# kyegomez/Kosmos-X

Measured on AMD Instinct MI355X. Metric: multimodal forward samples/sec (224x224 img + 50 tok) @ 24L/2048d, higher is better.
Workload: dtype mixed fp16/f16c (CLIP tower: fp16 MFMA; Perceiver + decoder: fp16 MFMA + fp8-e4m3 correction MFMAs; fp32 accumulate / residual / statistics)

## Files before the change

### include/kosmosx_hip.h

```cpp
#ifndef KOSMOSX_HIP_H
#define KOSMOSX_HIP_H

#include <stddef.h>
#include <stdint.h>

#ifdef __cplusplus
extern "C" {
#endif

#define KX_ABI_VERSION 7

typedef enum {
  KX_OK = 0,
  KX_ERR_INVALID_ARG = 1,
  KX_ERR_WORKSPACE = 2,
  KX_ERR_LAUNCH = 3,
  KX_ERR_UNSUPPORTED = 4
} kx_status;

typedef enum { KX_PREC_BF16 = 0, KX_PREC_F32 = 1, KX_PREC_BF16X3 = 2, KX_PREC_F16C = 3, KX_PREC_F16 = 4, KX_PREC_F32W24 = 5,
               KX_PREC_F32W16 = 6, KX_PREC_F16CHL = 7  } kx_precision;
typedef enum { KX_CORR_BOTH = 0, KX_CORR_WEIGHT = 1, KX_CORR_ACT = 2, KX_CORR_NONE = 3 } kx_f16c_corr;
typedef enum { KX_F32 = 0, KX_BF16 = 1, KX_BF16X3 = 2, KX_F16C = 3, KX_F16 = 4, KX_F16P = 5, KX_F16HL = 6 } kx_dtype;
typedef enum { KX_ACT_NONE = 0, KX_ACT_GELU = 1, KX_ACT_QUICK_GELU = 2, KX_ACT_RELU = 5, KX_ACT_SWISH = 6 } kx_act;
typedef enum { KX_ATTN_FULL = 0, KX_ATTN_CAUSAL = 1 } kx_attn_mask;

int kx_version(void);
int kx_last_error(char* buf, size_t n);


int kx_layernorm(const float* x, const float* pre_add, const float* gamma, const float* beta,
                 void* y, kx_dtype ydt, int64_t rows, int64_t cols, float eps,
                 int64_t rows_per_group, int64_t out_group_stride, int64_t out_row_offset,
                 void* stream);

typedef struct {
  const void* A; int64_t lda;
  const void* W; int64_t ldw;
  void* C; int64_t ldc; int32_t cdt;
  const float* bias;
  const float* residual; int64_t ldr;
  int64_t M, N, K;
  int32_t act;
  float qscale; int64_t qcols;
  const float* xq_cs; const float* xq_ss;
  const float* xk_cs; const float* xk_ss;
  int64_t xpos_T; int64_t xpos_dim;
  int32_t prec;
  int32_t tile;
  const float* row_stats; const float* colsum;
  float* stats_out;
  void* splitk_ws; size_t splitk_ws_bytes; int32_t splitk;
  const float* ln_gamma; const float* ln_beta; float ln_eps;
  const float* stats_partials; int64_t stats_in_nseg; int64_t stats_in_seg; float stats_eps;
  int32_t stats_out_seg;
  void* ln_out; int32_t ln_out_dt; const float* ln_out_gamma; const float* ln_out_beta; float ln_out_eps;
  const uint8_t* w_scale;
  void* ln_operand_out; int32_t ln_operand_dt; float* ln_operand_stats;
  int32_t w_tiled;
  int32_t ksplit; void* C2; const float* residual2; const float* a_add;
  void* pair_ws; size_t pair_ws_bytes;
  float* row_stats_scratch;
  int32_t f16c_corr;
  uint32_t* splitk_flags;
} kx_gemm_args;
int kx_gemm(const kx_gemm_args* args, void* stream);
int kx_pair_split_errors(unsigned* word_out);

typedef struct {
  const void* q; int64_t q_batch_stride; int64_t q_row_stride;
  const void* k; const void* v; int64_t kv_batch_stride; int64_t kv_row_stride;
  void* out; int64_t out_batch_stride; int64_t out_row_stride; int32_t odt;
  int64_t B, H, Tq, Tk;
  int32_t mask;
  int32_t prec;
  float* stats_out;
  float* lse_out;
  float dropout_p; int32_t dropout_site; uint64_t dropout_seed;
} kx_attn_args;
int kx_attention(const kx_attn_args* args, void* stream);

int kx_row_stats_finalize(const float* partials, int64_t rows, int64_t nseg, int64_t seg_size, float eps,
                          float* out, void* stream);

int kx_embed_splice(const int64_t* tokens, const float* embed, const float* pos, const float* img,
                    float* out, int64_t B, int64_t Tt, int64_t n_img, int64_t d, int64_t vocab,
                    int64_t max_pos, int64_t splice_at, int32_t u1_alias, int64_t pos_offset, void* stream);

int kx_token_range(const int64_t* tokens, int64_t n, int64_t* out2, void* stream);


typedef struct {
  uint32_t struct_bytes;
  int32_t do_sample;
  const float* logits; int64_t ld; int64_t B; int64_t V;
  float temperature; int32_t top_k; float top_p; float repetition_penalty;
  uint64_t seed; int64_t position;
  const int64_t* sequence_ids;
  int64_t* history; int64_t hist_ld; int64_t hist_len;
  uint8_t* finished;
  int64_t eos_id; int64_t pad_id;
  int64_t* next_token;
  int64_t* out_tokens; int64_t out_ld; int64_t out_col;
  int32_t* kept_count; uint8_t* keep_mask;
} kx_sample_args;
int kx_sample_logits(const kx_sample_args* args, void* stream);

int kx_embed_step(const int64_t* tokens, const float* embed, const float* pos, float* out, int64_t B, int64_t d,
                  int64_t vocab, int64_t max_pos, int64_t pos_a, int64_t pos_b, void* stream);

typedef enum {
  KX_STRUCT_GEMM_ARGS = 0, KX_STRUCT_ATTN_ARGS = 1, KX_STRUCT_VIT_LAYER = 2, KX_STRUCT_VIT_WEIGHTS = 3,
  KX_STRUCT_PERCEIVER_LAYER = 4, KX_STRUCT_PERCEIVER_WEIGHTS = 5, KX_STRUCT_DECODER_LAYER = 6,
  KX_STRUCT_DECODER_WEIGHTS = 7, KX_STRUCT_RESAMPLE_PLAN = 8, KX_STRUCT_PROF_RECORD = 9, KX_STRUCT_SAMPLE_ARGS = 10,
  KX_STRUCT_COUNT = 11
} kx_struct_id;
size_t kx_struct_bytes(int32_t id);
typedef struct {
  const float *ln1_g, *ln1_b;
  const void* wqkv; const float* bqkv;
  const void* wo;   const float* bo;
  const float *ln2_g, *ln2_b;
  const void* w1;   const float* b1;
  const void* w2;   const float* b2;
  const void* wqkv_f; const float* bqkv_f; const float* wqkv_colsum;
  const void* w1_f;   const float* b1_f;   const float* w1_colsum;
} kx_vit_layer;

typedef struct {
  uint32_t struct_bytes, layer_bytes;
  int32_t image, patch, dim, heads, ffn, layers, act; float eps;
  int32_t kpad;
  const void* wpatch;
  const float* cls;
  const float* pos;
  const float *pre_g, *pre_b;
  const kx_vit_layer* layer;
} kx_vit_weights;

size_t kx_vit_workspace_bytes(const kx_vit_weights* w, int64_t B, int32_t prec);
int kx_vit_forward(const kx_vit_weights* w, const float* pixels, int64_t B, float* out,
                   void* workspace, size_t workspace_bytes, int32_t prec, void* stream);

typedef struct {
  const float *nm_g, *nm_b, *nl_g, *nl_b;
  const void *wq, *wkv, *wout;
  const float *ff_g, *ff_b;
  const void *w1, *w2;
} kx_perceiver_layer;

typedef struct {
  uint32_t struct_bytes, layer_bytes;
  int32_t dim, depth, heads, latents, ff_mult, out_dim; float eps;
  const float* latents_p;
  const float* media_pos;
  const kx_perceiver_layer* layer;
  const float *norm_g, *norm_b;
  const void* wproj;
} kx_perceiver_weights;

size_t kx_perceiver_workspace_bytes(const kx_perceiver_weights* w, int64_t B, int64_t m, int32_t prec);
int kx_perceiver_forward(const kx_perceiver_weights* w, const float* x, int64_t B, int64_t m,
                         float* out, float* lat_out, void* workspace, size_t workspace_bytes,
// ... 148 lines not shown
```

### kosmos-x_amd/csrc/kx_attention.hip

```cpp
#include "kx_common.h"
#include "kx_dropout.h"

namespace {

__device__ __forceinline__ float score_nan_to_num(float s) {
  s = __builtin_isnan(s) ? 0.f : s;
  return fminf(fmaxf(s, -3.402823466e38f), 3.402823466e38f);
}

struct AttnParams {
  const char* q; long long qbs, qrs;
  const char* k; const char* v; long long kbs, krs;
  void* out; long long obs, ors; int o_bf16, o_x3, o_f16c;
  int B, H, Tq, Tk;
  float* stats_out;
  float* lse_out;
  float drop_inv_keep; unsigned drop_thresh; unsigned long long drop_seed; unsigned drop_site;
  int interleave;
};

constexpr int KSTR = 72;

template <bool CAUSAL>
__global__ __launch_bounds__(256) void attn_bf16_kernel(const AttnParams p) {
// ... 283 lines not shown
        const u32x4_t ones = (u32x4_t){ONE2, ONE2, ONE2, ONE2};
#pragma unroll
        for (int qb = 0; qb < 2; ++qb)
#pragma unroll
          for (int c = 0; c < 2; ++c)
            lt[qb] = mma16<F16>(ones, pf[qb][c], lt[qb]);
      }
      if (DROP) {
#pragma unroll
        for (int qb = 0; qb < 2; ++qb) {
          const unsigned long long row = (((unsigned long long)b * p.H + h) * p.Tq + (unsigned)(qw0 + qb * 16 + li)) * (unsigned long long)p.Tk;
#pragma unroll
          for (int kb = 0; kb < 4; ++kb) {
            const unsigned keep = kx_dropout_keep4_at(p.drop_seed, p.drop_site, row + (unsigned)(kv0 + kb * 16 + 4 * g), p.drop_thresh, (p.Tk & 3) != 0);
#pragma unroll
            for (int r = 0; r < 4; ++r) st[qb][kb][r] = ((keep >> r) & 1u) ? st[qb][kb][r] : 0.f;
          }
#pragma unroll
          for (int c = 0; c < 2; ++c) {
            pf[qb][c][0] = pack16x2<F16>(st[qb][2 * c][0], st[qb][2 * c][1]);
            pf[qb][c][1] = pack16x2<F16>(st[qb][2 * c][2], st[qb][2 * c][3]);
            pf[qb][c][2] = pack16x2<F16>(st[qb][2 * c + 1][0], st[qb][2 * c + 1][1]);
            pf[qb][c][3] = pack16x2<F16>(st[qb][2 * c + 1][2], st[qb][2 * c + 1][3]);
          }
        }
      }
#pragma unroll
      for (int d = 0; d < 4; ++d)
#pragma unroll
        for (int c = 0; c < 2; ++c) {
          const bf16_t* vr = &Vs[buf][(32 * c + 4 * g + (li >> 2)) * VSTR + d * 16 + (li & 3) * 4];
          const s16x4_t lo = __builtin_amdgcn_ds_read_tr16_b64_v4i16((lds_s16x4_t*)vr);
          const s16x4_t hi = __builtin_amdgcn_ds_read_tr16_b64_v4i16((lds_s16x4_t*)(vr + 16 * VSTR));
          const u32x2_t lo2 = __builtin_bit_cast(u32x2_t, lo), hi2 = __builtin_bit_cast(u32x2_t, hi);
          const u32x4_t vf = (u32x4_t){lo2[0], lo2[1], hi2[0], hi2[1]};
#pragma unroll
          for (int qb = 0; qb < 2; ++qb)
            ot[qb][d] = mma16<F16>(vf, pf[qb][c], ot[qb][d]);
        }
    }
    if (t + 1 < ntiles) lstore(buf ^ 1);
    __syncthreads();
  }
#pragma unroll
  for (int qb = 0; qb < 2; ++qb) {
    const float l = lt[qb][0];
    const float inv = (DROP ? p.drop_inv_keep : 1.0f) / l;
    const int qi = wave_live ? qw0 + qb * 16 + li : p.Tq;
    if (p.lse_out && g == 0 && qi < p.Tq)
      p.lse_out[((long long)b * p.H + h) * p.Tq + qi] = m_run[qb] + logf(l);
    if (p.stats_out) {
      float sm = 0.f;
#pragma unroll
      for (int d = 0; d < 4; ++d) sm += (ot[qb][d][0] + ot[qb][d][1]) + (ot[qb][d][2] + ot[qb][d][3]);
      sm *= inv;
      sm += __shfl_xor(sm, 16, 64);
      sm += __shfl_xor(sm, 32, 64);
      const float mu = sm * (1.0f / 64.0f);
      float m2 = 0.f;
#pragma unroll
      for (int d = 0; d < 4; ++d)
#pragma unroll
        for (int r = 0; r < 4; ++r) { const float dv = ot[qb][d][r] * inv - mu; m2 += dv * dv; }
      m2 += __shfl_xor(m2, 16, 64);
      m2 += __shfl_xor(m2, 32, 64);
      if (g == 0 && qi < p.Tq)
        *reinterpret_cast<float2*>(p.stats_out + 2 * (((long long)b * p.Tq + qi) * p.H + h)) = make_float2(sm, m2);
    }
    if (qi < p.Tq) {
      const long long ooff = (long long)b * p.obs + (long long)qi * p.ors + (long long)h * 64 + 4 * g;
#pragma unroll
      for (int d = 0; d < 4; ++d) {
        const float o0 = ot[qb][d][0] * inv, o1 = ot[qb][d][1] * inv, o2 = ot[qb][d][2] * inv, o3 = ot[qb][d][3] * inv;
        if (p.o_bf16) {
          uint2 pk; pk.x = pack16x2<F16>(o0, o1); pk.y = pack16x2<F16>(o2, o3);
          *reinterpret_cast<uint2*>(reinterpret_cast<bf16_t*>(p.out) + ooff + d * 16) = pk;
        } else {
          *reinterpret_cast<float4*>(reinterpret_cast<float*>(p.out) + ooff + d * 16) = make_float4(o0, o1, o2, o3);
        }
      }
    }
  }
  }
}


__device__ __forceinline__ void split_f16x8(const float (&x)[8], u32x4_t& hi, u32x4_t& lo) {
#pragma unroll
  for (int j = 0; j < 4; ++j) {
    const kx_f16x2_t h = __builtin_convertvector((kx_f32x2_t){clamp_f16(x[2 * j]), clamp_f16(x[2 * j + 1])}, kx_f16x2_t);
    hi[j] = __builtin_bit_cast(unsigned, h);
    lo[j] = pack_f16x2(x[2 * j] - (float)h[0], x[2 * j + 1] - (float)h[1]);
  }
}
__device__ __forceinline__ void split_f16x8_unit(const float (&x)[8], u32x4_t& hi, u32x4_t& lo) {
#pragma unroll
  for (int j = 0; j < 4; ++j) {
    const unsigned h = __builtin_bit_cast(unsigned, __builtin_convertvector((kx_f32x2_t){x[2 * j], x[2 * j + 1]}, kx_f16x2_t));
    unsigned l;
    asm("v_fma_mixlo_f16 %0, -%1, 1.0, %2 op_sel_hi:[1,0,0]" : "=v"(l) : "v"(h), "v"(x[2 * j]));
    asm("v_fma_mixhi_f16 %0, -%1, 1.0, %2 op_sel:[1,0,0] op_sel_hi:[1,0,0]" : "+v"(l) : "v"(h), "v"(x[2 * j + 1]));
    hi[j] = h; lo[j] = l;
  }
}
__device__ __forceinline__ f32x4_t mma_f16(u32x4_t a, u32x4_t b, f32x4_t c) {
  return __builtin_amdgcn_mfma_f32_16x16x32_f16(__builtin_bit_cast(f16x8_t, a), __builtin_bit_cast(f16x8_t, b), c, 0, 0, 0);
}

template <bool CAUSAL, int PVS, bool HL = false>
__global__ __launch_bounds__(256, 2) void attn_f16s_kernel(const AttnParams p) {
  __shared__ __attribute__((aligned(16))) unsigned short Kh[2][64 * 64], Kl[2][64 * 64];
  __shared__ __attribute__((aligned(16))) unsigned short Vh[2][64 * VSTR], Vl[2][64 * VSTR];
  constexpr float SC = 256.0f;
  const int tid = threadIdx.x, lane = tid & 63;
  const int wave = __builtin_amdgcn_readfirstlane(tid >> 6);
  const int g = lane >> 4, li = lane & 15;
  const int h = blockIdx.x, b = blockIdx.z;
  const int nx = (p.Tq + 127) >> 7;
  const int qb_second = nx - 1 - (int)blockIdx.y;
  const int npass = (CAUSAL && qb_second > (int)blockIdx.y) ? 2 : 1;
  for (int pass = 0; pass < npass; ++pass) {
  const int qblk0 = (pass == 0 ? (int)blockIdx.y : qb_second) * 128;
  const bool il = CAUSAL && p.interleave;
  const int qw0 = qblk0 + wave * 32;
  const int qrow[2] = {il ? qblk0 + wave * 16 : qw0, il ? qblk0 + 64 + wave * 16 : qw0 + 16};
  const bool wave_live = qrow[0] < p.Tq;
  const float* qp = reinterpret_cast<const float*>(p.q) + (long long)b * p.qbs + (long long)h * 64;
  const float* kp = reinterpret_cast<const float*>(p.k) + (long long)b * p.kbs + (long long)h * 64;
  const float* vp = reinterpret_cast<const float*>(p.v) + (long long)b * p.kbs + (long long)h * 64;

  u32x4_t qh[2][2], ql[2][2];
#pragma unroll
  for (int qb = 0; qb < 2; ++qb) {
    const float* qr = qp + (long long)min(qrow[qb] + li, p.Tq - 1) * p.qrs + 8 * g;
#pragma unroll
    for (int ks = 0; ks < 2; ++ks) {
      if constexpr (HL) {
        const char* slot = reinterpret_cast<const char*>(qr - 8 * g) + (32 * ks + 8 * g) * 2;
        qh[qb][ks] = *reinterpret_cast<const u32x4_t*>(slot);
        ql[qb][ks] = *reinterpret_cast<const u32x4_t*>(slot + 128);
      } else {
      const float4 a = *reinterpret_cast<const float4*>(qr + 32 * ks), c = *reinterpret_cast<const float4*>(qr + 32 * ks + 4);
      const float x[8] = {a.x * SC, a.y * SC, a.z * SC, a.w * SC, c.x * SC, c.y * SC, c.z * SC, c.w * SC};
      split_f16x8(x, qh[qb][ks], ql[qb][ks]);
      }
    }
  }
  f32x4_t ot[2][4];
  float m_run[2], l_run[2];
#pragma unroll
  for (int qb = 0; qb < 2; ++qb) {
    m_run[qb] = -INFINITY; l_run[qb] = 0.f;
#pragma unroll
    for (int d = 0; d < 4; ++d) ot[qb][d] = (f32x4_t){0.f, 0.f, 0.f, 0.f};
  }
  int ntiles = (p.Tk + 63) >> 6;
  if (CAUSAL) ntiles = min(ntiles, (min(qblk0 + 127, p.Tq - 1) >> 6) + 1);

  float4 kreg[2][2], vreg[2][2];
  u32x4_t kpc[2][2], vpc[2][2];
  auto gload = [&](int t) {
#pragma unroll
    for (int j = 0; j < 2; ++j) {
      const int c = tid + 256 * j, row = c >> 3, part = c & 7;
      if constexpr (HL) {
        const long long off = (long long)min(t * 64 + row, p.Tk - 1) * p.krs;
// ... 329 lines not shown
#pragma unroll
      for (int s2 = 0; s2 < 16; ++s2) st[kb] = __builtin_amdgcn_mfma_f32_16x16x4f32(kf[s2], qf[s2], st[kb], 0, 0, 0);
    }
    float mloc = -INFINITY;
#pragma unroll
    for (int kb = 0; kb < 4; ++kb)
#pragma unroll
      for (int r = 0; r < 4; ++r) {
        const int key = kv0 + kb * 16 + 4 * g + r;
        const bool ok = key < p.Tk && (!CAUSAL || key <= qi);
        st[kb][r] = ok ? (CAUSAL ? score_nan_to_num(st[kb][r]) : st[kb][r]) : -INFINITY;
        mloc = fmaxf(mloc, st[kb][r]);
      }
    mloc = fmaxf(mloc, __shfl_xor(mloc, 16, 64));
    mloc = fmaxf(mloc, __shfl_xor(mloc, 32, 64));
    const float m_new = fmaxf(m_run, mloc);
    const float m_safe = m_new == -INFINITY ? 0.f : m_new;
    const float alpha = expf(m_run - m_safe);
    float psum = 0.f;
#pragma unroll
    for (int kb = 0; kb < 4; ++kb)
#pragma unroll
      for (int r = 0; r < 4; ++r) {
        st[kb][r] = expf(st[kb][r] - m_safe);
        psum += st[kb][r];
      }
    l_run = l_run * alpha + psum;
    m_run = m_new;
#pragma unroll
    for (int d = 0; d < 4; ++d) ot[d] *= alpha;
#pragma unroll
    for (int kb = 0; kb < 4; ++kb)
#pragma unroll
      for (int r = 0; r < 4; ++r) {
        const float* vr = &Vs[(kb * 16 + 4 * g + r) * PITCH + li];
#pragma unroll
        for (int d = 0; d < 4; ++d) ot[d] = __builtin_amdgcn_mfma_f32_16x16x4f32(vr[d * 16], st[kb][r], ot[d], 0, 0, 0);
      }
  }
  l_run += __shfl_xor(l_run, 16, 64);
  l_run += __shfl_xor(l_run, 32, 64);
  const float inv = 1.0f / l_run;
  if (p.lse_out && g == 0 && qi < p.Tq) p.lse_out[((long long)b * p.H + h) * p.Tq + qi] = m_run + logf(l_run);
#pragma unroll
  for (int d = 0; d < 4; ++d) { ot[d][0] *= inv; ot[d][1] *= inv; ot[d][2] *= inv; ot[d][3] *= inv; }
  if (p.stats_out) {
    float sm = 0.f;
#pragma unroll
    for (int d = 0; d < 4; ++d) sm += (ot[d][0] + ot[d][1]) + (ot[d][2] + ot[d][3]);
    sm += __shfl_xor(sm, 16, 64); sm += __shfl_xor(sm, 32, 64);
    const float mu = sm * (1.0f / 64.0f);
    float m2 = 0.f;
#pragma unroll
    for (int d = 0; d < 4; ++d)
#pragma unroll
      for (int r = 0; r < 4; ++r) { const float dv = ot[d][r] - mu; m2 += dv * dv; }
    m2 += __shfl_xor(m2, 16, 64); m2 += __shfl_xor(m2, 32, 64);
    if (g == 0 && qi < p.Tq)
      *reinterpret_cast<float2*>(p.stats_out + 2 * (((long long)b * p.Tq + qi) * p.H + h)) = make_float2(sm, m2);
  }
  if (qi < p.Tq) {
    const long long ooff = (long long)b * p.obs + (long long)qi * p.ors + (long long)h * 64 + 4 * g;
#pragma unroll
    for (int d = 0; d < 4; ++d) {
      if (p.o_x3) {
        uint2 hh, ll;
        split_bf16x2(ot[d][0], ot[d][1], hh.x, ll.x); split_bf16x2(ot[d][2], ot[d][3], hh.y, ll.y);
        bf16_t* c = reinterpret_cast<bf16_t*>(p.out) + ooff + d * 16;
        const long long D = (long long)p.H * 64;
        *reinterpret_cast<uint2*>(c) = hh;
        *reinterpret_cast<uint2*>(c + D) = hh;
        *reinterpret_cast<uint2*>(c + 2 * D) = ll;
      } else if (p.o_bf16) {
        uint2 pk; pk.x = pack_bf16x2(ot[d][0], ot[d][1]); pk.y = pack_bf16x2(ot[d][2], ot[d][3]);
        *reinterpret_cast<uint2*>(reinterpret_cast<bf16_t*>(p.out) + ooff + d * 16) = pk;
      } else {
        *reinterpret_cast<float4*>(reinterpret_cast<float*>(p.out) + ooff + d * 16) =
            make_float4(ot[d][0], ot[d][1], ot[d][2], ot[d][3]);
      }
    }
  }
}

}

extern "C" int kx_attention(const kx_attn_args* a, void* stream) {
  KX_REQUIRE(a != nullptr, "kx_attention: null args");
  KX_REQUIRE(a->q && a->k && a->v && a->out, "kx_attention: null pointer");
  KX_REQUIRE(a->B > 0 && a->H > 0 && a->Tq > 0 && a->Tk > 0, "kx_attention: empty problem");
  KX_REQUIRE(a->H < 65536 && a->B < 65536, "kx_attention: B/H exceed the grid limits");
  KX_REQUIRE(a->mask != KX_ATTN_CAUSAL || a->Tq == a->Tk, "kx_attention: the causal mask needs Tq == Tk");
  KX_REQUIRE(a->prec == KX_PREC_BF16 || a->prec == KX_PREC_F32 || a->prec == KX_PREC_F16C || a->prec == KX_PREC_F16 || a->prec == KX_PREC_F16CHL,
             "kx_attention: bad precision");
  const bool f16 = a->prec == KX_PREC_F16;
  const int es = (a->prec == KX_PREC_BF16 || f16) ? 2 : 4;
  KX_REQUIRE(!f16 || ((a->odt == KX_F16 || a->odt == KX_F32) && !a->lse_out), "kx_attention: KX_PREC_F16 writes KX_F16 or fp32 (no lse)");
  KX_REQUIRE(a->odt != KX_F16 || f16, "kx_attention: a KX_F16 output comes from KX_PREC_F16");
  KX_REQUIRE((a->q_row_stride * es) % 16 == 0 && (a->kv_row_stride * es) % 16 == 0 &&
                 (a->q_batch_stride * es) % 16 == 0 && (a->kv_batch_stride * es) % 16 == 0,
             "kx_attention: strides must keep 16-byte alignment");
  KX_REQUIRE((((uintptr_t)a->q | (uintptr_t)a->k | (uintptr_t)a->v | (uintptr_t)a->out) & 15) == 0,
             "kx_attention: pointers must be 16-byte aligned");
  KX_REQUIRE(a->out_row_stride % 4 == 0 && a->out_batch_stride % 4 == 0, "kx_attention: output strides % 4");
  AttnParams p;
  p.q = (const char*)a->q; p.qbs = a->q_batch_stride; p.qrs = a->q_row_stride;
  p.k = (const char*)a->k; p.v = (const char*)a->v; p.kbs = a->kv_batch_stride; p.krs = a->kv_row_stride;
  p.out = a->out; p.obs = a->out_batch_stride; p.ors = a->out_row_stride; p.o_bf16 = a->odt == KX_BF16 || a->odt == KX_F16;
  p.o_x3 = a->odt == KX_BF16X3;
  p.o_f16c = a->odt == KX_F16C;
  const bool f16c_any = a->prec == KX_PREC_F16C || a->prec == KX_PREC_F16CHL;
  KX_REQUIRE(!p.o_f16c || (f16c_any && a->out_row_stride >= 2 * a->H * 64),
             "kx_attention: a KX_F16C output is produced by the KX_PREC_F16C kernel (row stride >= 2*H*64 2-byte units)");
  KX_REQUIRE(!f16c_any || a->odt == KX_F16C || a->odt == KX_F32, "kx_attention: KX_PREC_F16C writes KX_F16C or fp32");
  KX_REQUIRE(a->prec != KX_PREC_F16CHL || (!a->lse_out && a->dropout_p == 0.f), "kx_attention: KX_PREC_F16CHL is the forward kernel only");
  KX_REQUIRE(!p.o_x3 || (a->prec == KX_PREC_F32 && kx_tuning_get(KX_TUNE_ATTN_VARIANT) != 1 &&
                         a->out_row_stride >= 3 * a->H * 64),
             "kx_attention: a KX_BF16X3 output is produced by the fp32 matrix-core kernel only (row stride >= 3*H*64)");
  p.B = (int)a->B; p.H = (int)a->H; p.Tq = (int)a->Tq; p.Tk = (int)a->Tk;
  p.stats_out = a->stats_out;
  p.lse_out = a->lse_out;
  p.interleave = kx_tuning_get(KX_TUNE_ATTN_VARIANT) != 8;
  const bool drop = a->dropout_p > 0.f;
  const bool drop_mfma = drop && a->prec == KX_PREC_BF16 && kx_tuning_get(KX_TUNE_ATTN_VARIANT) != 1;
  KX_REQUIRE(a->dropout_p >= 0.f && a->dropout_p < 1.f && (!drop || ((a->prec == KX_PREC_F32 || drop_mfma) && a->odt == KX_F32 && !a->stats_out)),
             "kx_attention: dropout_p must be in [0, 1) and needs fp32 or bf16 q/k/v, an fp32 output and no stats_out");
  p.drop_thresh = drop ? (unsigned)fminf(4294967295.0f, a->dropout_p * 4294967296.0f) : 0u;
  p.drop_inv_keep = 1.0f / (1.0f - a->dropout_p);
  p.drop_seed = a->dropout_seed; p.drop_site = (unsigned)a->dropout_site;
  KX_REQUIRE(!a->lse_out || drop || kx_tuning_get(KX_TUNE_ATTN_VARIANT) != 1 || a->prec == KX_PREC_F32,
             "kx_attention: lse_out is not produced by the first-version (A/B) bf16 kernel");
  KX_REQUIRE(!a->stats_out || !(a->prec == KX_PREC_BF16 && kx_tuning_get(KX_TUNE_ATTN_VARIANT) == 1),
             "kx_attention: stats_out is not implemented by the v1 A/B kernel");
  hipStream_t s = (hipStream_t)stream;
  KxProfScope prof(a->prec == KX_PREC_F32 ? KX_K_ATTN_F32 : f16c_any ? KX_K_ATTN_F16S
                   : a->prec == KX_PREC_F16 ? KX_K_ATTN_F16 : KX_K_ATTN_BF16, a->B * a->H, a->Tq, a->Tk, s);
  const bool fold = a->mask != KX_ATTN_CAUSAL && a->Tq > 128 && (a->Tq - 1) % 128 < 32 && kx_tuning_get(KX_TUNE_ATTN_VARIANT) == 5;
  if (a->prec == KX_PREC_F16CHL) {
    const unsigned nx = (unsigned)((a->Tq + 127) / 128);
    const dim3 gc((unsigned)a->H, (nx + 1) / 2, (unsigned)a->B), gf((unsigned)a->H, nx, (unsigned)a->B);
    const int av = kx_tuning_get(KX_TUNE_ATTN_VARIANT);
    if (a->mask == KX_ATTN_CAUSAL) {
      if (av == 6) hipLaunchKernelGGL((attn_f16s_kernel<true, 2, true>), gc, dim3(256), 0, s, p);
      else if (av == 7) hipLaunchKernelGGL((attn_f16s_kernel<true, 3, true>), gc, dim3(256), 0, s, p);
      else hipLaunchKernelGGL((attn_f16s_kernel<true, 1, true>), gc, dim3(256), 0, s, p);
    } else hipLaunchKernelGGL((attn_f16s_kernel<false, 1, true>), gf, dim3(256), 0, s, p);
  } else if (a->prec == KX_PREC_F16C) {
    const unsigned nx = (unsigned)((a->Tq + 127) / 128);
    const int av = kx_tuning_get(KX_TUNE_ATTN_VARIANT);
    const dim3 gc((unsigned)a->H, (nx + 1) / 2, (unsigned)a->B), gf((unsigned)a->H, nx, (unsigned)a->B);
    if (a->mask == KX_ATTN_CAUSAL) {
      if (av == 4) hipLaunchKernelGGL((attn_f16s_kernel<true, 0>), gc, dim3(256), 0, s, p);
      else if (av == 6) hipLaunchKernelGGL((attn_f16s_kernel<true, 2>), gc, dim3(256), 0, s, p);
      else if (av == 7) hipLaunchKernelGGL((attn_f16s_kernel<true, 3>), gc, dim3(256), 0, s, p);
      else hipLaunchKernelGGL((attn_f16s_kernel<true, 1>), gc, dim3(256), 0, s, p);
    } else {
      if (av == 4) hipLaunchKernelGGL((attn_f16s_kernel<false, 0>), gf, dim3(256), 0, s, p);
      else hipLaunchKernelGGL((attn_f16s_kernel<false, 1>), gf, dim3(256), 0, s, p);
    }
  } else if (f16) {
    const unsigned nx = (unsigned)((a->Tq + 127) / 128);
    if (a->mask == KX_ATTN_CAUSAL)
      hipLaunchKernelGGL((attn_bf16_v2_kernel<true, true>), dim3((unsigned)a->H, (nx + 1) / 2, (unsigned)a->B), dim3(256), 0, s, p);
    else if (fold)
      hipLaunchKernelGGL((attn_bf16_v2_kernel<false, true, true>), dim3((unsigned)a->H, nx - 1, (unsigned)a->B), dim3(320), 0, s, p);
    else
      hipLaunchKernelGGL((attn_bf16_v2_kernel<false, true>), dim3((unsigned)a->H, nx, (unsigned)a->B), dim3(256), 0, s, p);
  } else if (a->prec == KX_PREC_BF16 && kx_tuning_get(KX_TUNE_ATTN_VARIANT) == 1) {
    dim3 grid((unsigned)((a->Tq + 63) / 64), (unsigned)a->H, (unsigned)a->B);
    if (a->mask == KX_ATTN_CAUSAL) hipLaunchKernelGGL(attn_bf16_kernel<true>, grid, dim3(256), 0, s, p);
    else hipLaunchKernelGGL(attn_bf16_kernel<false>, grid, dim3(256), 0, s, p);
  } else if (drop_mfma) {
    const unsigned nx = (unsigned)((a->Tq + 127) / 128);
    if (a->mask == KX_ATTN_CAUSAL)
      hipLaunchKernelGGL((attn_bf16_v2_kernel<true, false, false, true>), dim3((unsigned)a->H, (nx + 1) / 2, (unsigned)a->B), dim3(256), 0, s, p);
    else
      hipLaunchKernelGGL((attn_bf16_v2_kernel<false, false, false, true>), dim3((unsigned)a->H, nx, (unsigned)a->B), dim3(256), 0, s, p);
  } else if (a->prec == KX_PREC_BF16) {
    const unsigned nx = (unsigned)((a->Tq + 127) / 128);
    if (a->mask == KX_ATTN_CAUSAL)
      hipLaunchKernelGGL((attn_bf16_v2_kernel<true, false>), dim3((unsigned)a->H, (nx + 1) / 2, (unsigned)a->B), dim3(256), 0, s, p);
    else if (fold)
      hipLaunchKernelGGL((attn_bf16_v2_kernel<false, false, true>), dim3((unsigned)a->H, nx - 1, (unsigned)a->B), dim3(320), 0, s, p);
    else
      hipLaunchKernelGGL((attn_bf16_v2_kernel<false, false>), dim3((unsigned)a->H, nx, (unsigned)a->B), dim3(256), 0, s, p);
  } else if (kx_tuning_get(KX_TUNE_ATTN_VARIANT) != 1 && !drop) {
    dim3 grid((unsigned)((a->Tq + 63) / 64), (unsigned)a->H, (unsigned)a->B);
    if (a->mask == KX_ATTN_CAUSAL) hipLaunchKernelGGL(attn_f32_mfma_kernel<true>, grid, dim3(256), 0, s, p);
    else hipLaunchKernelGGL(attn_f32_mfma_kernel<false>, grid, dim3(256), 0, s, p);
  } else {
    dim3 grid((unsigned)((a->Tq + 3) / 4), (unsigned)a->H, (unsigned)a->B);
    const size_t lds = 4 * (64 + (size_t)a->Tk) * sizeof(float);
    KX_REQUIRE(lds <= 64 * 1024, "kx_attention(f32): Tk=%lld exceeds the LDS score buffer", (long long)a->Tk);
    if (a->mask == KX_ATTN_CAUSAL) hipLaunchKernelGGL(attn_f32_kernel<true>, grid, dim3(256), lds, s, p);
    else hipLaunchKernelGGL(attn_f32_kernel<false>, grid, dim3(256), lds, s, p);
  }
  KX_CHECK_LAUNCH("kx_attention");
  return KX_OK;
}

namespace {

struct DecodeParams {
  const char* qkv; long long qkv_row;
  char* kcache; char* vcache;
  long long cache_batch, cache_head, cache_row;
  void* out; long long out_row; int o_bf16, o_f16c, o_pieces;
  float* stats_out;
  int H, D, t;
};

template <typename T> struct Ld4;
template <> struct Ld4<bf16_t> {
  typedef uint2 raw;
  static constexpr int UK = 16;
  static __device__ __forceinline__ void unpack(const raw v, float (&x)[4]) {
    x[0] = __uint_as_float(v.x << 16); x[1] = __uint_as_float(v.x & 0xffff0000u);
    x[2] = __uint_as_float(v.y << 16); x[3] = __uint_as_float(v.y & 0xffff0000u);
  }
};
template <> struct Ld4<float> {
// ... 165 lines not shown
```

### kosmos-x_amd/kosmosx/_hip.py

```python
from __future__ import annotations

import ctypes as C
import logging
import os
from pathlib import Path

_LIB_PATH = Path(__file__).resolve().parent / "lib" / "libkosmosx_hip.so"
_lib = None
ABI_VERSION = 7

KX_PREC_BF16, KX_PREC_F32, KX_PREC_BF16X3, KX_PREC_F16C, KX_PREC_F16, KX_PREC_F32W24, KX_PREC_F32W16, KX_PREC_F16CHL = 0, 1, 2, 3, 4, 5, 6, 7
KX_F32, KX_BF16, KX_BF16X3, KX_F16C, KX_F16, KX_F16P, KX_F16HL = 0, 1, 2, 3, 4, 5, 6
KX_ACT_NONE, KX_ACT_GELU, KX_ACT_QUICK_GELU = 0, 1, 2
KX_ATTN_FULL, KX_ATTN_CAUSAL = 0, 1
KX_ACT_RELU, KX_ACT_SWISH = 5, 6
ACTS = {"none": KX_ACT_NONE, "gelu": KX_ACT_GELU, "quick_gelu": KX_ACT_QUICK_GELU, "relu": KX_ACT_RELU, "swish": KX_ACT_SWISH}
PRECS = {"bf16": KX_PREC_BF16, "fp32": KX_PREC_F32, "bf16x3": KX_PREC_BF16X3, "f16c": KX_PREC_F16C, "f16": KX_PREC_F16}
MODEL_PRECS = list(PRECS) + ["mixed"]
PACK_PRECS = dict(PRECS, w24=KX_PREC_F32, w16=KX_PREC_F32)


def stage_precision(prec: str, stage: str, widths=()) -> str:
    if prec == "mixed":
        if stage == "vit":
# ... 34 lines not shown
                                  "w1", "b1", "w2", "b2", "wqkv_f", "bqkv_f", "wqkv_colsum", "w1_f", "b1_f", "w1_colsum")]


class _SizedWeights(C.Structure):
    _layer_cls = None

    def __init__(self, *a, **k):
        super().__init__(*a, **k)
        self.struct_bytes, self.layer_bytes = C.sizeof(type(self)), C.sizeof(self._layer_cls)


class VitWeights(_SizedWeights):
    _layer_cls = VitLayer
    _fields_ = [("struct_bytes", C.c_uint32), ("layer_bytes", C.c_uint32), ("image", i32), ("patch", i32), ("dim", i32), ("heads", i32), ("ffn", i32), ("layers", i32),
                ("act", i32), ("eps", f32), ("kpad", i32),
                ("wpatch", vp), ("cls", vp), ("pos", vp), ("pre_g", vp), ("pre_b", vp),
                ("layer", C.POINTER(VitLayer))]


class PerceiverLayer(C.Structure):
    _fields_ = [(n, vp) for n in ("nm_g", "nm_b", "nl_g", "nl_b", "wq", "wkv", "wout", "ff_g", "ff_b", "w1", "w2")]


class PerceiverWeights(_SizedWeights):
    _layer_cls = PerceiverLayer
    _fields_ = [("struct_bytes", C.c_uint32), ("layer_bytes", C.c_uint32), ("dim", i32), ("depth", i32), ("heads", i32), ("latents", i32), ("ff_mult", i32), ("out_dim", i32),
                ("eps", f32), ("latents_p", vp), ("media_pos", vp), ("layer", C.POINTER(PerceiverLayer)),
                ("norm_g", vp), ("norm_b", vp), ("wproj", vp)]


class DecoderLayer(C.Structure):
    _fields_ = [(n, vp) for n in ("sa_g", "sa_b", "wqkv", "bqkv", "wo", "bo", "wo_colsum", "fl_g", "fl_b",
                                  "w1", "b1", "w2", "b2", "w2_colsum", "wqkv_f", "bqkv_f", "wqkv_colsum",
                                  "w1_f", "b1_f", "w1_colsum", "wqkv_t", "wo_t", "w1_t", "w2_t")]


class DecoderWeights(_SizedWeights):
    _layer_cls = DecoderLayer
    _fields_ = [("struct_bytes", C.c_uint32), ("layer_bytes", C.c_uint32), ("layers", i32), ("dim", i32), ("heads", i32), ("ffn", i32), ("vocab", i32), ("act", i32),
                ("subln", i32), ("xpos", i32), ("eps", f32), ("layer", C.POINTER(DecoderLayer)),
                ("ln_g", vp), ("ln_b", vp), ("wout", vp), ("wout_f", vp), ("bout_f", vp), ("wout_colsum", vp),
                ("wout_t", vp)]


class ProfRecord(C.Structure):
    _fields_ = [("kind", i32), ("reserved", i32), ("a", i64), ("b", i64), ("c", i64), ("ms", f32),
                ("reserved2", f32)]


class ResamplePlan(C.Structure):
    _fields_ = [("crop", i32), ("hk", i32), ("vk", i32), ("y_first", i32), ("rows_needed", i32), ("x_first", i32),
                ("span_px", i32), ("hbounds", vp), ("hcoef", vp), ("vbounds", vp), ("vcoef", vp)]


class SampleArgs(C.Structure):
    _fields_ = [("struct_bytes", C.c_uint32), ("do_sample", i32), ("logits", vp), ("ld", i64), ("B", i64), ("V", i64),
                ("temperature", f32), ("top_k", i32), ("top_p", f32), ("repetition_penalty", f32),
                ("seed", C.c_uint64), ("position", i64), ("sequence_ids", vp),
                ("history", vp), ("hist_ld", i64), ("hist_len", i64), ("finished", vp), ("eos_id", i64), ("pad_id", i64),
                ("next_token", vp), ("out_tokens", vp), ("out_ld", i64), ("out_col", i64),
                ("kept_count", vp), ("keep_mask", vp)]

    def __init__(self, *a, **k):
        super().__init__(*a, **k)
        self.struct_bytes = C.sizeof(type(self))


KERNEL_KINDS = ["gemm_bf16_128x128", "gemm_bf16_64x64", "gemm_f32_128x128", "gemm_f32_64x64", "layernorm",
                "attn_bf16", "attn_f32", "embed", "misc", "gemm_bf16_160x128", "gemm_bf16_256x128_phased",
                "gemm_bf16_256x256_phased",
                "gemm_f16c_128x128", "gemm_f16c_64x64", "gemm_f16c_160x128", "gemm_f16c_256x128_phased", "gemm_f16c_256x256_phased",
                "gemm_f16_128x128", "gemm_f16_64x64", "gemm_f16_160x128", "gemm_f16_256x128_phased", "gemm_f16_256x256_phased",
                "attn_f16", "attn_f16s"]


SYMBOLS = {
    "kx_version": (C.c_int, []),
    "kx_last_error": (C.c_int, [C.c_char_p, C.c_size_t]),
    "kx_struct_bytes": (C.c_size_t, [i32]),
    "kx_layernorm": (C.c_int, [vp, vp, vp, vp, vp, C.c_int, i64, i64, f32, i64, i64, i64, vp]),
    "kx_gemm": (C.c_int, [C.POINTER(GemmArgs), vp]),
    "kx_pair_split_errors": (C.c_int, [C.POINTER(C.c_uint)]),
    "kx_attention": (C.c_int, [C.POINTER(AttnArgs), vp]),
    "kx_row_stats_finalize": (C.c_int, [vp, i64, i64, i64, f32, vp, vp]),
    "kx_embed_splice": (C.c_int, [vp, vp, vp, vp, vp, i64, i64, i64, i64, i64, i64, i64, i32, i64, vp]),
    "kx_token_range": (C.c_int, [vp, i64, vp, vp]),
    "kx_sample_logits": (C.c_int, [C.POINTER(SampleArgs), vp]),
    "kx_embed_step": (C.c_int, [vp, vp, vp, vp, i64, i64, i64, i64, i64, i64, vp]),
    "kx_set_tuning": (C.c_int, [C.c_int, C.c_int]),
    "kx_prof_enable": (C.c_int, [C.c_int]),
    "kx_prof_collect": (C.c_int, [C.POINTER(ProfRecord), C.c_int]),
    "kx_vit_workspace_bytes": (C.c_size_t, [C.POINTER(VitWeights), i64, i32]),
    "kx_vit_forward": (C.c_int, [C.POINTER(VitWeights), vp, i64, vp, vp, C.c_size_t, i32, vp]),
    "kx_perceiver_workspace_bytes": (C.c_size_t, [C.POINTER(PerceiverWeights), i64, i64, i32]),
    "kx_perceiver_forward": (C.c_int, [C.POINTER(PerceiverWeights), vp, i64, i64, vp, vp, vp, C.c_size_t, i32, vp]),
    "kx_decoder_workspace_bytes": (C.c_size_t, [C.POINTER(DecoderWeights), i64, i64, i32]),
    "kx_decoder_prefill": (C.c_int, [C.POINTER(DecoderWeights), vp, i64, i64, vp, vp, vp, vp, vp, i32, vp, vp, i64, vp,
                                     C.c_size_t, i32, vp]),
    "kx_decoder_decode_step": (C.c_int, [C.POINTER(DecoderWeights), vp, i64, i64, vp, vp, vp, vp, vp, vp, i64, vp, i32,
                                         vp, C.c_size_t, i32, vp]),
    "kx_attention_decode": (C.c_int, [vp, vp, vp, vp, i32, vp, i64, i64, i64, i64, i32, vp]),
    "kx_decoder_forward": (C.c_int, [C.POINTER(DecoderWeights), vp, i64, i64, vp, vp, vp, vp, vp, i32, vp,
                                     C.c_size_t, i32, vp]),
    "kx_clip_preprocess_workspace_bytes": (C.c_size_t, [i64, i32, i32]),
    "kx_clip_preprocess": (C.c_int, [vp, i64, i32, i32, i64, i64, C.POINTER(ResamplePlan), vp, vp, vp, vp,
                                     C.c_size_t, vp]),
    "kx_token_splice": (C.c_int, [vp, i64, i64, i64, i64, i64, i64, vp, vp, vp]),
    "kx_transpose": (C.c_int, [vp, vp, i64, i64, i64, i64, i32, vp]),
    "kx_to_operand": (C.c_int, [vp, vp, i64, i64, i64, i64, i32, i32, vp]),
    "kx_to_operand_pair_workspace_bytes": (C.c_size_t, [i64, i64]),
    "kx_to_operand_pair": (C.c_int, [vp, vp, vp, i64, i64, i64, i64, i64, vp, vp, C.c_size_t, vp]),
    "kx_gelu_backward_operand_pair": (C.c_int, [vp, vp, vp, vp, i64, i64, i64, i64, i64, vp, vp, C.c_size_t, vp]),
    "kx_colsum_workspace_bytes": (C.c_size_t, [i64, i64]),
    "kx_colsum": (C.c_int, [vp, i64, i64, i64, vp, i32, vp, C.c_size_t, vp]),
    "kx_layernorm_backward_workspace_bytes": (C.c_size_t, [i64, i64]),
    "kx_layernorm_backward": (C.c_int, [vp, vp, vp, vp, vp, vp, vp, i64, i64, f32, vp, C.c_size_t, vp]),
    "kx_gelu_layernorm": (C.c_int, [vp, vp, vp, vp, C.c_int, i64, i64, f32, vp]),
    "kx_gelu_layernorm_backward_supported": (C.c_int, [i64]),
    "kx_gelu_layernorm_backward": (C.c_int, [vp, vp, vp, vp, vp, vp, vp, i64, i64, f32, vp, C.c_size_t, vp]),
    "kx_gelu_forward": (C.c_int, [vp, vp, i64, vp]),
    "kx_gelu_backward": (C.c_int, [vp, vp, vp, i64, vp]),
    "kx_cross_entropy": (C.c_int, [vp, i64, i64, i64, vp, f32, vp, vp, i64, vp]),
    "kx_reduce_sum": (C.c_int, [vp, i64, i32, vp, i32, vp, C.c_size_t, vp]),
    "kx_xpos_backward": (C.c_int, [vp, i64, i64, i64, vp, vp, vp, vp, f32, vp]),
    "kx_embed_backward": (C.c_int, [vp, vp, i64, i64, i64, i64, i64, vp, vp, vp]),
    "kx_adamw": (C.c_int, [vp, vp, vp, vp, i64, f32, f32, f32, f32, f32, i64, vp, f32, vp]),
    "kx_lion": (C.c_int, [vp, vp, vp, i64, f32, f32, f32, f32, vp, f32, vp]),
    "kx_attention_backward_dropout": (C.c_int, [vp] * 10 + [i64] * 7 + [i32, f32, C.c_uint64, i32, vp]),
    "kx_attention_backward_dropout_bf16": (C.c_int, [vp] * 3 + [i32] + [vp] * 7 + [i64] * 7 + [i32, f32, C.c_uint64, i32, vp]),
    "kx_dropout": (C.c_int, [vp, vp, vp, i64, f32, C.c_uint64, i32, vp]),
    "kx_dropout_mask": (C.c_int, [vp, i64, f32, C.c_uint64, i32, vp]),
    "kx_quick_gelu_forward": (C.c_int, [vp, vp, i64, vp]),
    "kx_quick_gelu_backward": (C.c_int, [vp, vp, vp, i64, vp]),
    "kx_add_rowvec": (C.c_int, [vp, vp, vp, i64, i64, vp]),
    "kx_patchify": (C.c_int, [vp, vp, i64, i32, i32, i32, i32, vp]),
    "kx_vit_assemble": (C.c_int, [vp, vp, vp, vp, i64, i32, i32, vp]),
    "kx_attention_backward": (C.c_int, [vp, vp, vp, i32] + [vp] * 7 + [i64] * 7 + [i32, i32, vp]),
}


STRUCT_IDS = [GemmArgs, AttnArgs, VitLayer, VitWeights, PerceiverLayer, PerceiverWeights, DecoderLayer, DecoderWeights,
              ResamplePlan, ProfRecord, SampleArgs]


def lib_path() -> Path:
    return Path(os.environ.get("KOSMOSX_HIP_LIB", str(_LIB_PATH)))


def load():
    global _lib
    if _lib is not None:
        return _lib
    path = lib_path()
    if not path.exists():
        msg = (f"libkosmosx_hip.so not found at {path}: build it with `python kosmos-x_amd/build.py` "
               "(hipcc --offload-arch=gfx950). The Kosmos-X MI355X path has no CPU fallback.")
        logging.error(msg)
        raise RuntimeError(msg)
    try:
        lib = C.CDLL(str(path))
    except OSError as e:
        logging.error(f"Failed to load {path}: {e}")
        raise RuntimeError(f"Failed to load {path}: {e}") from e
    for name, (res, args) in SYMBOLS.items():
        fn = getattr(lib, name)
        fn.restype, fn.argtypes = res, args
# ... 41 lines not shown
```

Measured before the change: 1348.

## Add whole-head attention kernel staging all K/V in LDS once per head

```diff
diff --git a/include/kosmosx_hip.h b/include/kosmosx_hip.h
--- a/include/kosmosx_hip.h
+++ b/include/kosmosx_hip.h
@@ -79,6 +79,7 @@
   float dropout_p; int32_t dropout_site; uint64_t dropout_seed;
 } kx_attn_args;
 int kx_attention(const kx_attn_args* args, void* stream);
+int kx_attention_whole_head(const kx_attn_args* args);
 
 int kx_row_stats_finalize(const float* partials, int64_t rows, int64_t nseg, int64_t seg_size, float eps,
                           float* out, void* stream);
diff --git a/kosmos-x_amd/csrc/kx_attention.hip b/kosmos-x_amd/csrc/kx_attention.hip
--- a/kosmos-x_amd/csrc/kx_attention.hip
+++ b/kosmos-x_amd/csrc/kx_attention.hip
@@ -389,6 +389,234 @@
     }
   }
   }
+}
+
+constexpr int WH_MAX_TK = 272;
+
+template <bool F16>
+__device__ __forceinline__ unsigned pack16x2_unit(float lo, float hi) {
+  if constexpr (F16) return __builtin_bit_cast(unsigned, __builtin_convertvector((kx_f32x2_t){lo, hi}, kx_f16x2_t));
+  else return pack_bf16x2(lo, hi);
+}
+
+template <bool F16>
+__device__ __forceinline__ void wh_load_q(const bf16_t* qp, const AttnParams& p, int qrow0, int g, int li, u32x4_t (&qf)[2][2]) {
+#pragma unroll
+  for (int qb = 0; qb < 2; ++qb) {
+    const bf16_t* qr = qp + (long long)min(qrow0 + qb * 16 + li, p.Tq - 1) * p.qrs + 8 * g;
+    qf[qb][0] = *reinterpret_cast<const u32x4_t*>(qr);
+    qf[qb][1] = *reinterpret_cast<const u32x4_t*>(qr + 32);
+  }
+}
+
+template <bool F16, int NQ>
+__device__ __forceinline__ void wh_pass(const AttnParams& p, const bf16_t* Ks, const bf16_t* Vs, const u32x4_t (&qf)[2][2],
+                                        int b, int h, int qrow0, int g, int li) {
+  f32x4_t ot[NQ][4];
+  float m_run[NQ];
+  f32x4_t lt[NQ];
+#pragma unroll
+  for (int qb = 0; qb < NQ; ++qb) {
+    m_run[qb] = -INFINITY; lt[qb] = (f32x4_t){0.f, 0.f, 0.f, 0.f};
+#pragma unroll
+    for (int d = 0; d < 4; ++d) ot[qb][d] = (f32x4_t){0.f, 0.f, 0.f, 0.f};
+  }
+  auto step = [&](auto last_c, int kv0) __attribute__((always_inline)) {
+    constexpr bool LAST = decltype(last_c)::value;
+    const int nkb = LAST ? min(4, (p.Tk - kv0 + 15) >> 4) : 4;
+    f32x4_t st[NQ][4];
+#pragma unroll
+    for (int kb = 0; kb < 4; ++kb) {
+      if (!LAST || kb < nkb) {
+        const int krow = kv0 + kb * 16 + li;
+#pragma unroll
+        for (int qb = 0; qb < NQ; ++qb) st[qb][kb] = (f32x4_t){0.f, 0.f, 0.f, 0.f};
+#pragma unroll
+        for (int ks = 0; ks < 2; ++ks) {
+          const u32x4_t kf = *reinterpret_cast<const u32x4_t*>(&Ks[krow * 64 + (((ks * 4 + g) ^ (krow & 7)) << 3)]);
+#pragma unroll
+          for (int qb = 0; qb < NQ; ++qb) st[qb][kb] = mma16<F16>(kf, qf[qb][ks], st[qb][kb]);
+        }
+      } else {
+#pragma unroll
+        for (int qb = 0; qb < NQ; ++qb) st[qb][kb] = (f32x4_t){-INFINITY, -INFINITY, -INFINITY, -INFINITY};
+      }
+    }
+    if constexpr (NQ == 2)
+      asm volatile("s_nop 7\n\ts_nop 4" : "+v"(st[0][0]), "+v"(st[0][1]), "+v"(st[0][2]), "+v"(st[0][3]),
+                                          "+v"(st[1][0]), "+v"(st[1][1]), "+v"(st[1][2]), "+v"(st[1][3]));
+    else
+      asm volatile("s_nop 7\n\ts_nop 4" : "+v"(st[0][0]), "+v"(st[0][1]), "+v"(st[0][2]), "+v"(st[0][3]));
+    const bool need_mask = LAST && (kv0 + 63 >= p.Tk);
+    u32x4_t pf[NQ][2];
+    float mneg[NQ], alpha[NQ];
+    constexpr float LOG2E = 1.44269504088896340736f;
+#pragma unroll
+    for (int qb = 0; qb < NQ; ++qb) {
+      if (need_mask) {
+#pragma unroll
+        for (int kb = 0; kb < 4; ++kb)
+#pragma unroll
+          for (int r = 0; r < 4; ++r) {
+            const int key = kv0 + kb * 16 + 4 * g + r;
+            st[qb][kb][r] = key < p.Tk ? st[qb][kb][r] : -INFINITY;
+          }
+      }
+      const float a0 = max3_raw(st[qb][0][0], st[qb][0][1], st[qb][0][2]);
+      const float a1 = max3_raw(st[qb][1][0], st[qb][1][1], st[qb][1][2]);
+      const float a2 = max3_raw(st[qb][2][0], st[qb][2][1], st[qb][2][2]);
+      const float a3 = max3_raw(st[qb][3][0], st[qb][3][1], st[qb][3][2]);
+      const float b0 = max3_raw(a0, st[qb][0][3], st[qb][1][3]);
+      const float b1 = max3_raw(a1, st[qb][2][3], st[qb][3][3]);
+      const float c0 = max3_raw(b0, a2, a3);
+      const float m_new = quad_max(max3_raw(c0, b1, m_run[qb]), m_run[qb]);
+      mneg[qb] = -m_new * LOG2E;
+      alpha[qb] = __builtin_amdgcn_exp2f(fmaf(m_run[qb], LOG2E, mneg[qb]));
+      m_run[qb] = m_new;
+    }
+    bool same = alpha[0] == 1.0f;
+    if constexpr (NQ == 2) same = same && alpha[1] == 1.0f;
+    if (!__all(same)) {
+#pragma unroll
+      for (int qb = 0; qb < NQ; ++qb) {
+#pragma unroll
+        for (int d = 0; d < 4; ++d) ot[qb][d] *= alpha[qb];
+        lt[qb] *= alpha[qb];
+      }
+    }
+#pragma unroll
+    for (int qb = 0; qb < NQ; ++qb) {
+#pragma unroll
+      for (int kb = 0; kb < 4; ++kb)
+#pragma unroll
+        for (int r = 0; r < 4; ++r) st[qb][kb][r] = __builtin_amdgcn_exp2f(fmaf(st[qb][kb][r], LOG2E, mneg[qb]));
+#pragma unroll
+      for (int c = 0; c < 2; ++c) {
+        pf[qb][c][0] = pack16x2_unit<F16>(st[qb][2 * c][0], st[qb][2 * c][1]);
+        pf[qb][c][1] = pack16x2_unit<F16>(st[qb][2 * c][2], st[qb][2 * c][3]);
+        pf[qb][c][2] = pack16x2_unit<F16>(st[qb][2 * c + 1][0], st[qb][2 * c + 1][1]);
+        pf[qb][c][3] = pack16x2_unit<F16>(st[qb][2 * c + 1][2], st[qb][2 * c + 1][3]);
+      }
+    }
+    constexpr unsigned ONE2 = F16 ? 0x3c003c00u : 0x3f803f80u;
+    const u32x4_t ones = (u32x4_t){ONE2, ONE2, ONE2, ONE2};
+#pragma unroll
+    for (int c = 0; c < 2; ++c) {
+      if (LAST && 2 * c >= nkb) continue;
+#pragma unroll
+      for (int qb = 0; qb < NQ; ++qb) lt[qb] = mma16<F16>(ones, pf[qb][c], lt[qb]);
+    }
+#pragma unroll
+    for (int d = 0; d < 4; ++d)
+#pragma unroll
+      for (int c = 0; c < 2; ++c) {
+        if (LAST && 2 * c >= nkb) continue;
+        const bf16_t* vr = &Vs[(kv0 + 32 * c + 4 * g + (li >> 2)) * VSTR + d * 16 + (li & 3) * 4];
+        const u32x2_t lo2 = __builtin_bit_cast(u32x2_t, __builtin_amdgcn_ds_read_tr16_b64_v4i16((lds_s16x4_t*)vr));
+        u32x2_t hi2 = (u32x2_t){0u, 0u};
+        if (!LAST || 2 * c + 1 < nkb)
+          hi2 = __builtin_bit_cast(u32x2_t, __builtin_amdgcn_ds_read_tr16_b64_v4i16((lds_s16x4_t*)(vr + 16 * VSTR)));
+        const u32x4_t vf = (u32x4_t){lo2[0], lo2[1], hi2[0], hi2[1]};
+#pragma unroll
+        for (int qb = 0; qb < NQ; ++qb) ot[qb][d] = mma16<F16>(vf, pf[qb][c], ot[qb][d]);
+      }
+  };
+  const int nsteps = (p.Tk + 63) >> 6;
+  for (int t = 0; t + 1 < nsteps; ++t) step(std::integral_constant<bool, false>{}, t * 64);
+  step(std::integral_constant<bool, true>{}, (nsteps - 1) * 64);
+
+#pragma unroll
+  for (int qb = 0; qb < NQ; ++qb) {
+    const float l = lt[qb][0];
+    const float inv = 1.0f / l;
+    const int qi = qrow0 + qb * 16 + li;
+    if (p.stats_out) {
+      float sm = 0.f;
+#pragma unroll
+      for (int d = 0; d < 4; ++d) sm += (ot[qb][d][0] + ot[qb][d][1]) + (ot[qb][d][2] + ot[qb][d][3]);
+      sm *= inv;
+      sm += __shfl_xor(sm, 16, 64);
+      sm += __shfl_xor(sm, 32, 64);
+      const float mu = sm * (1.0f / 64.0f);
+      float m2 = 0.f;
+#pragma unroll
+      for (int d = 0; d < 4; ++d)
+#pragma unroll
+        for (int r = 0; r < 4; ++r) { const float dv = ot[qb][d][r] * inv - mu; m2 += dv * dv; }
+      m2 += __shfl_xor(m2, 16, 64);
+      m2 += __shfl_xor(m2, 32, 64);
+      if (g == 0 && qi < p.Tq)
+        *reinterpret_cast<float2*>(p.stats_out + 2 * (((long long)b * p.Tq + qi) * p.H + h)) = make_float2(sm, m2);
+    }
+    if (qi < p.Tq) {
+      const long long ooff = (long long)b * p.obs + (long long)qi * p.ors + (long long)h * 64 + 4 * g;
+#pragma unroll
+      for (int d = 0; d < 4; ++d) {
+        const float o0 = ot[qb][d][0] * inv, o1 = ot[qb][d][1] * inv, o2 = ot[qb][d][2] * inv, o3 = ot[qb][d][3] * inv;
+        if (p.o_bf16) {
+          uint2 pk; pk.x = pack16x2<F16>(o0, o1); pk.y = pack16x2<F16>(o2, o3);
+          *reinterpret_cast<uint2*>(reinterpret_cast<bf16_t*>(p.out) + ooff + d * 16) = pk;
+        } else {
+          *reinterpret_cast<float4*>(reinterpret_cast<float*>(p.out) + ooff + d * 16) = make_float4(o0, o1, o2, o3);
+        }
+      }
+    }
+  }
+}
+
+template <bool F16>
+__global__ __launch_bounds__(512, 4) void attn_wh16_kernel(const AttnParams p) {
+  constexpr int RC = WH_MAX_TK;
+  __shared__ __attribute__((aligned(16))) bf16_t Ks[RC * 64];
+  __shared__ __attribute__((aligned(16))) bf16_t Vs[RC * VSTR];
+  const int tid = threadIdx.x, lane = tid & 63;
+  const int wave = __builtin_amdgcn_readfirstlane(tid >> 6);
+  const int g = lane >> 4, li = lane & 15;
+  const int h = blockIdx.x, b = blockIdx.y;
+  const bf16_t* qp = reinterpret_cast<const bf16_t*>(p.q) + (long long)b * p.qbs + (long long)h * 64;
+  const bf16_t* kp = reinterpret_cast<const bf16_t*>(p.k) + (long long)b * p.kbs + (long long)h * 64;
+  const bf16_t* vp = reinterpret_cast<const bf16_t*>(p.v) + (long long)b * p.kbs + (long long)h * 64;
+
+  auto map_pass = [&](int q0, int n, int rot, int& row0, int& nblk) {
+    const int nb = (n + 15) >> 4;
+    if (nb <= 8) { const int j = (wave - rot) & 7; row0 = q0 + j * 16; nblk = j < nb ? 1 : 0; }
+    else { row0 = q0 + wave * 32; nblk = wave * 2 + 1 < nb ? 2 : wave * 2 < nb ? 1 : 0; }
+  };
+  const bool two = p.Tq > 256;
+  int rowa, nblka, rowt = 0, nblkt = 0;
+  const int wg = b * (int)gridDim.x + h;
+  map_pass(0, min(p.Tq, 256), 0, rowa, nblka);
+  if (two) map_pass(256, p.Tq - 256, ((wg >> 8) + (wg >> 3)) & 7, rowt, nblkt);
+  u32x4_t qa[2][2], qt[2][2];
+  if (nblkt) wh_load_q<F16>(qp, p, rowt, g, li, qt);
+  if (nblka) wh_load_q<F16>(qp, p, rowa, g, li, qa);
+
+  {
+    const int nchunk = ((p.Tk + 15) & ~15) * 8;
+    constexpr int NJ = (RC * 8 + 511) / 512;
+    u32x4_t kreg[NJ], vreg[NJ];
+#pragma unroll
+    for (int j = 0; j < NJ; ++j) {
+      const int c = min(tid + 512 * j, nchunk - 1), row = c >> 3, part = c & 7;
+      const long long off = (long long)min(row, p.Tk - 1) * p.krs + part * 8;
+      kreg[j] = *reinterpret_cast<const u32x4_t*>(kp + off);
+      vreg[j] = *reinterpret_cast<const u32x4_t*>(vp + off);
+    }
+#pragma unroll
+    for (int j = 0; j < NJ; ++j) {
+      const int c = tid + 512 * j, row = c >> 3, part = c & 7;
+      if (c < nchunk) {
+        *reinterpret_cast<u32x4_t*>(&Ks[row * 64 + ((part ^ (row & 7)) << 3)]) = kreg[j];
+        *reinterpret_cast<u32x4_t*>(&Vs[row * VSTR + part * 8]) = vreg[j];
+      }
+    }
+  }
+  __syncthreads();
+
+  if (nblkt == 2) wh_pass<F16, 2>(p, Ks, Vs, qt, b, h, rowt, g, li);
+  else if (nblkt == 1) wh_pass<F16, 1>(p, Ks, Vs, qt, b, h, rowt, g, li);
+  if (nblka == 2) wh_pass<F16, 2>(p, Ks, Vs, qa, b, h, rowa, g, li);
+  else if (nblka == 1) wh_pass<F16, 1>(p, Ks, Vs, qa, b, h, rowa, g, li);
 }
 
 
@@ -884,7 +1112,14 @@
   }
 }
 
-}
+bool attn_takes_whole_head(const kx_attn_args* a) {
+  return (a->prec == KX_PREC_BF16 || a->prec == KX_PREC_F16) && a->mask != KX_ATTN_CAUSAL && !(a->dropout_p > 0.f) &&
+         !a->lse_out && a->Tk <= WH_MAX_TK && a->Tq <= 512 && kx_tuning_get(KX_TUNE_ATTN_VARIANT) == 0;
+}
+
+}
+
+extern "C" int kx_attention_whole_head(const kx_attn_args* a) { return a != nullptr && attn_takes_whole_head(a) ? 1 : 0; }
 
 extern "C" int kx_attention(const kx_attn_args* a, void* stream) {
   KX_REQUIRE(a != nullptr, "kx_attention: null args");
@@ -937,7 +1172,11 @@
   KxProfScope prof(a->prec == KX_PREC_F32 ? KX_K_ATTN_F32 : f16c_any ? KX_K_ATTN_F16S
                    : a->prec == KX_PREC_F16 ? KX_K_ATTN_F16 : KX_K_ATTN_BF16, a->B * a->H, a->Tq, a->Tk, s);
   const bool fold = a->mask != KX_ATTN_CAUSAL && a->Tq > 128 && (a->Tq - 1) % 128 < 32 && kx_tuning_get(KX_TUNE_ATTN_VARIANT) == 5;
-  if (a->prec == KX_PREC_F16CHL) {
+  if (attn_takes_whole_head(a)) {
+    const dim3 gw((unsigned)a->H, (unsigned)a->B);
+    if (f16) hipLaunchKernelGGL((attn_wh16_kernel<true>), gw, dim3(512), 0, s, p);
+    else hipLaunchKernelGGL((attn_wh16_kernel<false>), gw, dim3(512), 0, s, p);
+  } else if (a->prec == KX_PREC_F16CHL) {
     const unsigned nx = (unsigned)((a->Tq + 127) / 128);
     const dim3 gc((unsigned)a->H, (nx + 1) / 2, (unsigned)a->B), gf((unsigned)a->H, nx, (unsigned)a->B);
     const int av = kx_tuning_get(KX_TUNE_ATTN_VARIANT);
diff --git a/kosmos-x_amd/kosmosx/_hip.py b/kosmos-x_amd/kosmosx/_hip.py
--- a/kosmos-x_amd/kosmosx/_hip.py
+++ b/kosmos-x_amd/kosmosx/_hip.py
@@ -140,6 +140,7 @@
     "kx_gemm": (C.c_int, [C.POINTER(GemmArgs), vp]),
     "kx_pair_split_errors": (C.c_int, [C.POINTER(C.c_uint)]),
     "kx_attention": (C.c_int, [C.POINTER(AttnArgs), vp]),
+    "kx_attention_whole_head": (C.c_int, [C.POINTER(AttnArgs)]),
     "kx_row_stats_finalize": (C.c_int, [vp, i64, i64, i64, f32, vp, vp]),
     "kx_embed_splice": (C.c_int, [vp, vp, vp, vp, vp, i64, i64, i64, i64, i64, i64, i64, i32, i64, vp]),
     "kx_token_range": (C.c_int, [vp, i64, vp, vp]),
```

After: 1348 (median of 4 runs). Within noise of the previous version (+0.0%).
